# WangWen-Believer/DR-SLAM

Measured on AMD Instinct MI355X. Metric: RGB-D frames/sec (extract+match) at 640x480, higher is better.
Workload: dtype u8; 1 GPU; 640x480 synthetic RGB-D (TUM3 intrinsics), ORB extract 1000/1.2/8/20/7 + SearchByProjection(frame k, frame k-1, th=15) on consecutive frames; BASELINE config 2; batch_per_gpu=512, batches_in_flight_per_gpu=3, distinct_resident_input_batches_per_gpu=3, sequence_frames_per_rank=64

## Files before the change

### dr_slam_amd/csrc/match_kernels.hip

```cpp
#include "drfe_internal.h"
#include "match_internal.h"
#include "../../include/drfe_math.h"

#define WAVE 64


__global__ __launch_bounds__(256) void k_undistort(const drfe_keypoint* __restrict__ kps, const int* __restrict__ kpCount,
                                                   int maxKp, DrfeDistortion D, drfe_keypoint* __restrict__ kpsUn)
{
    const int slot = blockIdx.y;
    const int i = blockIdx.x * 256 + threadIdx.x;
    if (i >= kpCount[slot]) return;
    drfe_keypoint kp = kps[(size_t)slot * maxKp + i];
    float ux, uy;
    drfe_undistort_point(D, kp.x, kp.y, &ux, &uy);
    kp.x = ux; kp.y = uy;
    kpsUn[(size_t)slot * maxKp + i] = kp;
}

__global__ __launch_bounds__(256) void k_stereo(const drfe_keypoint* __restrict__ kps, const drfe_keypoint* __restrict__ kpsUn,
                                                const int* __restrict__ kpCount,
                                                int maxKp, const uint16_t* __restrict__ depth, size_t frameStride,
                                                size_t rowStride, int w, int h, drfe_camera cam,
                                                float* __restrict__ uRight, float* __restrict__ zDepth)
{
    const int slot = blockIdx.y;
    const int i = blockIdx.x * 256 + threadIdx.x;
    if (i >= kpCount[slot]) return;
    const drfe_keypoint kp = kps[(size_t)slot * maxKp + i];
    const int v = (int)kp.y, u = (int)kp.x;
    float d = 0.f;
    if (u >= 0 && u < w && v >= 0 && v < h)
        d = (float)depth[rowStride ? (size_t)slot * frameStride + (size_t)v * rowStride + u : (size_t)slot * frameStride + i] * cam.depth_factor;
    float ur = -1.f, z = -1.f;
    if (d > 0) { z = d; ur = kpsUn[(size_t)slot * maxKp + i].x - cam.bf / d; }
    uRight[(size_t)slot * maxKp + i] = ur;
    zDepth[(size_t)slot * maxKp + i] = z;
}

__device__ __forceinline__ int grid_cell(const drfe_keypoint& kp, const drfe_camera& cam, float invW, float invH)
{
    const int px = (int)roundf((kp.x - cam.min_x) * invW);
    const int py = (int)roundf((kp.y - cam.min_y) * invH);
    if (px < 0 || px >= DRFE_GRID_COLS || py < 0 || py >= DRFE_GRID_ROWS) return -1;
    return px * DRFE_GRID_ROWS + py;
}

__global__ __launch_bounds__(256) void k_grid(const drfe_keypoint* __restrict__ kps, const int* __restrict__ kpCount,
                                              int maxKp, drfe_camera cam, float invW, float invH,
                                              const float* __restrict__ uRight, const uint8_t* __restrict__ desc,
                                              int* __restrict__ gridOff, int* __restrict__ gridIdx,
                                              uint4* __restrict__ cellKp, uint4* __restrict__ cellDesc)
{
    __shared__ int cnt[DRFE_GRID_CELLS];
    __shared__ int off[DRFE_GRID_CELLS + 1];
    __shared__ int part[256];
    const int slot = blockIdx.x, tid = threadIdx.x;
    const int n = kpCount[slot];
    const drfe_keypoint* K = kps + (size_t)slot * maxKp;
    int* gIdx = gridIdx + (size_t)slot * maxKp;
    int* gOff = gridOff + (size_t)slot * (DRFE_GRID_CELLS + 1);
    for (int c = tid; c < DRFE_GRID_CELLS; c += 256) cnt[c] = 0;
    __syncthreads();
    for (int i = tid; i < n; i += 256) {
        const int c = grid_cell(K[i], cam, invW, invH);
        if (c >= 0) atomicAdd(&cnt[c], 1);
    }
    __syncthreads();
    const int per = DRFE_GRID_CELLS / 256;
    int s = 0;
    for (int k = 0; k < per; k++) s += cnt[tid * per + k];
    part[tid] = s;
    __syncthreads();
    for (int o = 1; o < 256; o <<= 1) {
        const int v = (tid >= o) ? part[tid - o] : 0;
        __syncthreads();
        part[tid] += v;
        __syncthreads();
    }
    int run = part[tid] - s;
    for (int k = 0; k < per; k++) { off[tid * per + k] = run; run += cnt[tid * per + k]; }
    if (tid == 255) off[DRFE_GRID_CELLS] = run;
    __syncthreads();
    for (int c = tid; c <= DRFE_GRID_CELLS; c += 256) gOff[c] = off[c];
    for (int c = tid; c < DRFE_GRID_CELLS; c += 256) cnt[c] = 0;
    __syncthreads();
    for (int i = tid; i < n; i += 256) {
        const int c = grid_cell(K[i], cam, invW, invH);
        if (c >= 0) gIdx[off[c] + atomicAdd(&cnt[c], 1)] = i;
    }
    __syncthreads();
    for (int c = tid; c < DRFE_GRID_CELLS; c += 256) {
        const int b = off[c], e = off[c + 1];
        for (int a = b + 1; a < e; a++) {
            const int v = gIdx[a];
            int j = a - 1;
            while (j >= b && gIdx[j] > v) { gIdx[j + 1] = gIdx[j]; j--; }
            gIdx[j + 1] = v;
        }
    }
    __syncthreads();
    const int nIn = off[DRFE_GRID_CELLS];
    uint4* cK = cellKp + (size_t)slot * maxKp;
    uint4* cD = cellDesc + (size_t)slot * maxKp * 2;
    const uint4* D4 = reinterpret_cast<const uint4*>(desc + (size_t)slot * maxKp * 32);
    const float* UR = uRight + (size_t)slot * maxKp;
    for (int p = tid; p < nIn; p += 256) {
        const int idx = gIdx[p];
        const drfe_keypoint kp = K[idx];
        cK[p] = make_uint4(__float_as_uint(kp.x), __float_as_uint(kp.y), __float_as_uint(UR[idx]),
                           (uint32_t)idx | ((uint32_t)kp.octave << 24));
        cD[2 * p] = D4[2 * idx];
        cD[2 * p + 1] = D4[2 * idx + 1];
    }
}


__device__ __forceinline__ void mat3_mul_add(const float* T , const float x[3], float out[3])
{
#pragma unroll
    for (int r = 0; r < 3; r++) {
        const float d = T[r * 4 + 0] * x[0] + T[r * 4 + 1] * x[1] + T[r * 4 + 2] * x[2];
        out[r] = d + T[r * 4 + 3];
    }
}

__global__ __launch_bounds__(256) void k_mappoints_last(const drfe_keypoint* __restrict__ kps,
                                                        const uint8_t* __restrict__ desc,
                                                        const int* __restrict__ kpCount, int maxKp,
                                                        const float* __restrict__ zDepth, drfe_camera cam,
                                                        const float* __restrict__ Twc ,
                                                        drfe_map_point* __restrict__ mps)
{
    const int slot = blockIdx.y;
    const int i = blockIdx.x * 256 + threadIdx.x;
    if (i >= kpCount[slot]) return;
    const size_t o = (size_t)slot * maxKp + i;
    drfe_map_point mp;
    const float z = zDepth[o];
    mp.valid = z > 0 ? 1 : 0;
    mp.obs_positive = 1;
    mp.pad[0] = mp.pad[1] = 0;
    mp.world[0] = mp.world[1] = mp.world[2] = 0.f;
    if (z > 0) {
        const float invfx = 1.0f / cam.fx, invfy = 1.0f / cam.fy;
        const drfe_keypoint kp = kps[o];
        float p[3];
        p[0] = (kp.x - cam.cx) * z * invfx;
        p[1] = (kp.y - cam.cy) * z * invfy;
        p[2] = z;
        mat3_mul_add(Twc + (size_t)slot * 16, p, mp.world);
    }
    const uint32_t* d = reinterpret_cast<const uint32_t*>(desc + o * 32);
    uint32_t* md = reinterpret_cast<uint32_t*>(mp.desc);
#pragma unroll
    for (int k = 0; k < 8; k++) md[k] = d[k];
    mps[o] = mp;
}

__global__ __launch_bounds__(256) void k_queries_last(const MatchPair* __restrict__ pairs,
                                                      const drfe_keypoint* __restrict__ kps,
                                                      const int* __restrict__ kpCount, int maxKp,
                                                      const drfe_map_point* __restrict__ mps, drfe_camera cam,
                                                      const float* __restrict__ scaleFactors, float th,
                                                      MatchQuery* __restrict__ queries)
{
    const MatchPair P = pairs[blockIdx.y];
    const int i = blockIdx.x * 256 + threadIdx.x;
    const int nLast = P.mpSlot >= 0 ? kpCount[P.lastSlot] : P.nQueries;
    if (i >= nLast) return;
    MatchQuery q;
    q.valid = 0;
    q.u = q.v = q.radius = q.ur = q.thrR = 0.f;
    q.minLevel = q.maxLevel = -1;
    q.obs = 0;
    const drfe_map_point mp = mps[(size_t)P.mpBase + i];
#pragma unroll
    for (int k = 0; k < 8; k++) q.desc[k] = reinterpret_cast<const uint32_t*>(mp.desc)[k];
    q.obs = mp.obs_positive;
    if (mp.valid) {
        float xc[3];
        mat3_mul_add(P.Tcw, mp.world, xc);
        const float invzc = (float)(1.0 / (double)xc[2]);
        if (!(invzc < 0)) {
            const float u = cam.fx * xc[0] * invzc + cam.cx;
            const float v = cam.fy * xc[1] * invzc + cam.cy;
            if (!(u < cam.min_x || u > cam.max_x) && !(v < cam.min_y || v > cam.max_y)) {
                const int oct = kps[(size_t)P.lastSlot * maxKp + i].octave;
                const float radius = th * scaleFactors[oct];
                q.u = u; q.v = v; q.radius = radius; q.thrR = radius;
                q.ur = u - cam.bf * invzc;
                if (P.forward) { q.minLevel = oct; q.maxLevel = -1; }
                else if (P.backward) { q.minLevel = 0; q.maxLevel = oct; }
                else { q.minLevel = oct - 1; q.maxLevel = oct + 1; }
                q.valid = 1;
            }
        }
    }
    queries[(size_t)P.queryBase + i] = q;
}


__device__ __forceinline__ bool window_cells(const MatchQuery& q, const drfe_camera& cam, float invW, float invH, int& minX,
                                             int& maxX, int& minY, int& maxY)
{
    const float x = q.u, y = q.v, r = q.radius;
    minX = max(0, (int)floorf((x - cam.min_x - r) * invW));
    maxX = min(DRFE_GRID_COLS - 1, (int)ceilf((x - cam.min_x + r) * invW));
    minY = max(0, (int)floorf((y - cam.min_y - r) * invH));
    maxY = min(DRFE_GRID_ROWS - 1, (int)ceilf((y - cam.min_y + r) * invH));
    return !(minX >= DRFE_GRID_COLS || maxX < 0 || minY >= DRFE_GRID_ROWS || maxY < 0);
}

__device__ __forceinline__ bool window_candidate(const MatchQuery& q, bool bCheckLevels, const uint4* __restrict__ cK,
                                                 const uint4* __restrict__ cD, int p, int sq, uint64_t q0, uint64_t q1,
                                                 uint64_t q2, uint64_t q3, uint32_t& key, uint32_t& id)
{
    const uint4 k4 = cK[p];
    const uint4 da = cD[2 * p], db = cD[2 * p + 1];
    const float kx = __uint_as_float(k4.x), ky = __uint_as_float(k4.y), ur = __uint_as_float(k4.z);
    const int oct = (int)(k4.w >> 24);
    bool ok = true;
    if (bCheckLevels) {
        if (oct < q.minLevel) ok = false;
        if (q.maxLevel >= 0 && oct > q.maxLevel) ok = false;
    }
    const float dx = kx - q.u, dy = ky - q.v;
    if (!(fabsf(dx) < q.radius && fabsf(dy) < q.radius)) ok = false;
    if (ur > 0) {
        const float er = fabsf(q.ur - ur);
        if (er > q.thrR) ok = false;
    }
    if (!ok) return false;
    const int dist = __popcll(q0 ^ ((uint64_t)da.x | ((uint64_t)da.y << 32))) + __popcll(q1 ^ ((uint64_t)da.z | ((uint64_t)da.w << 32))) +
                     __popcll(q2 ^ ((uint64_t)db.x | ((uint64_t)db.y << 32))) + __popcll(q3 ^ ((uint64_t)db.z | ((uint64_t)db.w << 32)));
    key = ((uint32_t)dist << 22) | (uint32_t)min(sq, (1 << 22) - 1);
    id = k4.w;
    return true;
}

__device__ void window_query_wave(const MatchQuery& q, size_t qo, int lane, int nMinCellX, int nMaxCellX, int nMinCellY, int nMaxCellY,
                                  const int* __restrict__ gOff, const uint4* __restrict__ cK, const uint4* __restrict__ cD,
                                  uint32_t* __restrict__ candIdx, uint32_t* __restrict__ candKey, int* __restrict__ candCnt,
                                  uint2* __restrict__ candBest, int* __restrict__ status)
{
    const bool bCheckLevels = (q.minLevel > 0) || (q.maxLevel >= 0);
    uint32_t* oIdx = candIdx + qo * DRFE_MATCH_MAX_CAND;
    uint32_t* oKey = candKey + qo * DRFE_MATCH_MAX_CAND;
    const uint64_t q0 = (uint64_t)q.desc[0] | ((uint64_t)q.desc[1] << 32), q1 = (uint64_t)q.desc[2] | ((uint64_t)q.desc[3] << 32),
                   q2 = (uint64_t)q.desc[4] | ((uint64_t)q.desc[5] << 32), q3 = (uint64_t)q.desc[6] | ((uint64_t)q.desc[7] << 32);
    const int ncol = nMaxCellX - nMinCellX + 1;
    int runB = 0, runN = 0;
    if (lane < ncol) {
        const int cb = (nMinCellX + lane) * DRFE_GRID_ROWS;
        runB = gOff[cb + nMinCellY];
        runN = gOff[cb + nMaxCellY + 1] - runB;
    }
    const int incl = drfe_wave_incl_scan(runN, lane);
    const int T = __builtin_amdgcn_readlane(incl, 63);
    int nOut = 0;
    bool overflow = false;
    uint32_t myKey = 0xFFFFFFFFu, myIdx = 0;
    for (int s0 = 0; s0 < T; s0 += WAVE) {
        const int sq = s0 + lane;
        bool pass = false;
        uint32_t key = 0xFFFFFFFFu, id = 0;
        int base = __builtin_amdgcn_readfirstlane(runB);
        for (int j = 0; j + 1 < ncol; j++) {
            const int inclJ = __builtin_amdgcn_readlane(incl, j), nextB = __builtin_amdgcn_readlane(runB, j + 1);
            if (inclJ <= sq) base = nextB - inclJ;
        }
        if (sq < T) pass = window_candidate(q, bCheckLevels, cK, cD, base + sq, sq, q0, q1, q2, q3, key, id);
        const unsigned long long m = __ballot(pass);
        const int pos = nOut + __popcll(m & ((1ull << lane) - 1ull));
        if (pass) {
            if (pos < DRFE_MATCH_MAX_CAND) {
                oIdx[pos] = id;
                oKey[pos] = key;
                if (key < myKey) { myKey = key; myIdx = id; }
            } else overflow = true;
        }
        nOut += __popcll(m);
    }
    if (__any(overflow) && lane == 0) atomicOr(status, 4);
    const uint32_t mn = drfe_wave_min_u32(myKey);
    const unsigned long long who = __ballot(myKey == mn);
    const uint32_t bIdx = (uint32_t)__builtin_amdgcn_readlane((int)myIdx, __ffsll((long long)who) - 1);
    if (lane == 0) {
        candCnt[qo] = min(nOut, DRFE_MATCH_MAX_CAND);
        candBest[qo] = make_uint2(mn, bIdx);
    }
}

#define WQ_TAB 64
#ifndef WQ_THREADS
#define WQ_THREADS 64
#endif
#define WQ_PER_BLOCK (WQ_THREADS / WAVE * 4)
__global__ __launch_bounds__(WQ_THREADS) void k_window_candidates(const MatchPair* __restrict__ pairs,
                                                           const MatchQuery* __restrict__ queries,
                                                           const int* __restrict__ kpCount, int maxKp,
                                                           const int* __restrict__ gridOff,
                                                           const uint4* __restrict__ cellKp,
                                                           const uint4* __restrict__ cellDesc, drfe_camera cam,
                                                           float invW, float invH,
                                                           uint32_t* __restrict__ candIdx,
                                                           uint32_t* __restrict__ candKey,
                                                           int* __restrict__ candCnt, uint2* __restrict__ candBest,
                                                           int* __restrict__ status, uint32_t gxMagic)
{
    __shared__ int sTab[WQ_THREADS / WAVE][4][WQ_TAB];
    int bx, by;
    drfe_xcd_swizzle_2d(gxMagic, bx, by);
    const MatchPair P = pairs[by];
    const int wv = __builtin_amdgcn_readfirstlane((int)(threadIdx.x >> 6)), lane = threadIdx.x & 63;
    const int g = lane >> 4, l = lane & 15;
    const int qbase = (bx * (WQ_THREADS / WAVE) + wv) * 4;
    const int nQ = P.mpSlot >= 0 ? kpCount[P.lastSlot] : P.nQueries;
    if (qbase >= nQ) return;
    const int cur = P.curSlot;
    const int* gOff = gridOff + (size_t)cur * (DRFE_GRID_CELLS + 1);
    const uint4* cK = cellKp + (size_t)cur * maxKp;
    const uint4* cD = cellDesc + (size_t)cur * maxKp * 2;
    const bool have = qbase + g < nQ;
    const size_t qo = (size_t)P.queryBase + (have ? qbase + g : qbase);
    const MatchQuery q = queries[qo];
    int nMinCellX = 0, nMaxCellX = 0, nMinCellY = 0, nMaxCellY = 0;
    const bool inRange = have && q.valid && window_cells(q, cam, invW, invH, nMinCellX, nMaxCellX, nMinCellY, nMaxCellY);
    const int ncol = nMaxCellX - nMinCellX + 1;
    int runB = 0, runN = 0;
    const bool narrow = inRange && ncol <= 16;
    if (narrow && l < ncol) {
        const int cb = (nMinCellX + l) * DRFE_GRID_ROWS;
        runB = gOff[cb + nMinCellY];
        runN = gOff[cb + nMaxCellY + 1] - runB;
    }
    int incl = runN;
    incl += __builtin_amdgcn_update_dpp(0, incl, 0x111, 0xf, 0xf, true);
    incl += __builtin_amdgcn_update_dpp(0, incl, 0x112, 0xf, 0xf, true);
    incl += __builtin_amdgcn_update_dpp(0, incl, 0x114, 0xf, 0xf, true);
    incl += __builtin_amdgcn_update_dpp(0, incl, 0x118, 0xf, 0xf, true);
    const int T = __shfl(incl, 15, 16);
    const bool small = narrow && T <= WQ_TAB;
    {
        const int excl = incl - runN;
        const int n = small ? runN : 0;
        for (int k = 0; __any(k < n); k++)
            if (k < n) sTab[wv][g][excl + k] = runB + k;
    }
    const bool bCheckLevels = (q.minLevel > 0) || (q.maxLevel >= 0);
    const uint64_t q0 = (uint64_t)q.desc[0] | ((uint64_t)q.desc[1] << 32), q1 = (uint64_t)q.desc[2] | ((uint64_t)q.desc[3] << 32),
                   q2 = (uint64_t)q.desc[4] | ((uint64_t)q.desc[5] << 32), q3 = (uint64_t)q.desc[6] | ((uint64_t)q.desc[7] << 32);
    uint32_t* oIdx = candIdx + qo * DRFE_MATCH_MAX_CAND;
    uint32_t* oKey = candKey + qo * DRFE_MATCH_MAX_CAND;
    const int Tg = small ? T : 0;
    int nOut = 0;
    uint32_t myKey = 0xFFFFFFFFu, myIdx = 0;
    for (int s0 = 0; __any(s0 < Tg); s0 += 16) {
        const int sq = s0 + l;
        bool pass = false;
        uint32_t key = 0xFFFFFFFFu, id = 0;
        if (sq < Tg) pass = window_candidate(q, bCheckLevels, cK, cD, sTab[wv][g][sq], sq, q0, q1, q2, q3, key, id);
        const uint32_t m16 = (uint32_t)(__ballot(pass) >> (g * 16)) & 0xFFFFu;
        const int pos = nOut + __popc(m16 & ((1u << l) - 1u));
        if (pass) {
            oIdx[pos] = id;
            oKey[pos] = key;
            if (key < myKey) { myKey = key; myIdx = id; }
        }
        nOut += __popc(m16);
    }
    uint32_t mn = myKey;
    mn = min(mn, (uint32_t)__builtin_amdgcn_update_dpp((int)mn, (int)mn, 0xB1, 0xf, 0xf, false));
    mn = min(mn, (uint32_t)__builtin_amdgcn_update_dpp((int)mn, (int)mn, 0x4E, 0xf, 0xf, false));
    mn = min(mn, (uint32_t)__builtin_amdgcn_update_dpp((int)mn, (int)mn, 0x141, 0xf, 0xf, false));
    mn = min(mn, (uint32_t)__builtin_amdgcn_update_dpp((int)mn, (int)mn, 0x140, 0xf, 0xf, false));
    const uint32_t who16 = (uint32_t)(__ballot(myKey == mn) >> (g * 16)) & 0xFFFFu;
    const uint32_t bIdx = (uint32_t)__shfl((int)myIdx, __ffs((int)who16) - 1, 16);
    if (have && l == 0 && (small || !inRange)) {
        candCnt[qo] = nOut;
        candBest[qo] = small ? make_uint2(mn, bIdx) : make_uint2(0xFFFFFFFFu, 0u);
    }
    unsigned long long wide = __ballot(inRange && !small && l == 0);
    while (wide) {
        const int gg = (__ffsll((long long)wide) - 1) >> 4;
        wide &= wide - 1;
        const size_t qw = (size_t)P.queryBase + qbase + gg;
        const MatchQuery qq = queries[qw];
        int x0, x1, y0, y1;
        window_cells(qq, cam, invW, invH, x0, x1, y0, y1);
        window_query_wave(qq, qw, lane, x0, x1, y0, y1, gOff, cK, cD, candIdx, candKey, candCnt, candBest, status);
    }
}


__device__ __forceinline__ uint32_t wave_min_u32(uint32_t v) { return drfe_wave_min_u32(v); }

#define RS_THREADS 512
#define RS_MAX_T 8
static_assert(RS_THREADS * RS_MAX_T == DRFE_MATCH_LAST_MAX_QUERIES, "the C-ABI checks this limit before launching");
__global__ __launch_bounds__(RS_THREADS) void k_resolve_last(const MatchPair* __restrict__ pairs,
                                                             const MatchQuery* __restrict__ queries,
                                                             const drfe_keypoint* __restrict__ kps,
                                                             const int* __restrict__ kpCount, int maxKp,
                                                             const uint32_t* __restrict__ candIdx,
                                                             const uint32_t* __restrict__ candKey,
                                                             const int* __restrict__ candCnt,
                                                             const uint2* __restrict__ candBest, int checkOri,
                                                             int* __restrict__ match ,
                                                             const uint8_t* __restrict__ initObs,
                                                             int* __restrict__ matchCount,
                                                             uint16_t* __restrict__ histScratch )
{
    extern __shared__ int rs_smem[];
    int* owner = rs_smem;
    unsigned char* claim = reinterpret_cast<unsigned char*>(rs_smem + maxKp);
    __shared__ int hist[30];
    __shared__ int sNm, sEnt, sInd[3], sChanged[3];
    const MatchPair P = pairs[blockIdx.x];
    const int tid = threadIdx.x;
    const int nQ = P.mpSlot >= 0 ? kpCount[P.lastSlot] : P.nQueries;
    const int nCur = kpCount[P.curSlot];
    int* M = match + (size_t)P.curSlot * maxKp;
    const drfe_keypoint* Kc = kps + (size_t)P.curSlot * maxKp;
    const drfe_keypoint* Kl = kps + (size_t)P.lastSlot * maxKp;
    uint16_t* hs = histScratch + (size_t)blockIdx.x * 2 * maxKp;
    for (int i = tid; i < nCur; i += RS_THREADS) {
        unsigned char c = 0;
        if (M[i] >= 0) c = 1 | ((initObs ? initObs[i] : 1) ? 2 : 0);
        claim[i] = c;
    }
    if (tid < 30) hist[tid] = 0;
    if (tid == 0) { sNm = 0; sEnt = 0; sChanged[0] = 0; }
    const float factor = 1.0f / 30;
    int cnt[RS_MAX_T], obs[RS_MAX_T];
    uint32_t bKey[RS_MAX_T], bIdx[RS_MAX_T], pKey[RS_MAX_T], pIdx[RS_MAX_T];
#pragma unroll
    for (int t = 0; t < RS_MAX_T; t++) {
        const int i = tid + t * RS_THREADS;
        cnt[t] = 0; obs[t] = 0; bKey[t] = 0xFFFFFFFFu; bIdx[t] = 0; pKey[t] = 0xFFFFFFFFu; pIdx[t] = 0;
        if (i < nQ) {
            const size_t qo = (size_t)P.queryBase + i;
            cnt[t] = candCnt[qo];
            if (cnt[t] > 0) { const uint2 b = candBest[qo]; bKey[t] = b.x; bIdx[t] = b.y; obs[t] = queries[qo].obs; }
        }
    }
    for (int sweep = 0;; sweep++) {
        for (int k = tid; k < nCur; k += RS_THREADS) owner[k] = 0x7FFFFFFF;
        if (tid == 0) sChanged[(sweep + 1) % 3] = 0;
        __syncthreads();
#pragma unroll
        for (int t = 0; t < RS_MAX_T; t++)
            if (obs[t] && pKey[t] != 0xFFFFFFFFu && (int)(pKey[t] >> 22) <= 100)
                atomicMin(&owner[pIdx[t] & 0xFFFFFF], tid + t * RS_THREADS);
        __syncthreads();
        bool changed = false;
#pragma unroll
        for (int t = 0; t < RS_MAX_T; t++) {
            if (cnt[t] == 0) continue;
            const int i = tid + t * RS_THREADS;
            uint32_t key = 0xFFFFFFFFu, idx = 0;
            const int kb = (int)(bIdx[t] & 0xFFFFFF);
            if ((claim[kb] & 3) != 3 && owner[kb] >= i) { key = bKey[t]; idx = bIdx[t]; }
            else {
                const size_t qo = ((size_t)P.queryBase + i) * DRFE_MATCH_MAX_CAND;
                for (int j0 = 0; j0 < cnt[t]; j0 += 8) {
                    const uint4 ka = *reinterpret_cast<const uint4*>(candKey + qo + j0);
                    const uint4 kb2 = *reinterpret_cast<const uint4*>(candKey + qo + j0 + 4);
                    const uint4 ia = *reinterpret_cast<const uint4*>(candIdx + qo + j0);
                    const uint4 ib = *reinterpret_cast<const uint4*>(candIdx + qo + j0 + 4);
                    const uint32_t kv[8] = {ka.x, ka.y, ka.z, ka.w, kb2.x, kb2.y, kb2.z, kb2.w};
                    const uint32_t iv[8] = {ia.x, ia.y, ia.z, ia.w, ib.x, ib.y, ib.z, ib.w};
#pragma unroll
                    for (int u = 0; u < 8; u++) {
                        if (j0 + u >= cnt[t] || kv[u] >= key) continue;
                        const int kk = (int)(iv[u] & 0xFFFFFF);
                        if ((claim[kk] & 3) != 3 && owner[kk] >= i) { key = kv[u]; idx = iv[u]; }
                    }
                }
            }
            if (key != pKey[t] || idx != pIdx[t]) { changed = true; pKey[t] = key; pIdx[t] = idx; }
        }
        if (changed) sChanged[sweep % 3] = 1;
        __syncthreads();
        if (!__builtin_amdgcn_readfirstlane(sChanged[sweep % 3])) break;
    }
    for (int k = tid; k < nCur; k += RS_THREADS) owner[k] = -1;
    __syncthreads();
#pragma unroll
    for (int t = 0; t < RS_MAX_T; t++) {
        if (pKey[t] == 0xFFFFFFFFu || (int)(pKey[t] >> 22) > 100) continue;
        const int i = tid + t * RS_THREADS;
        const int i2 = (int)(pIdx[t] & 0xFFFFFF);
        atomicMax(&owner[i2], i);
        atomicAdd(&sNm, 1);
        if (checkOri) {
            float rot = Kl[i].angle - Kc[i2].angle;
            if (rot < 0.0f) rot += 360.0f;
            int bin = (int)roundf(rot * factor);
            if (bin == 30) bin = 0;
            const int e = atomicAdd(&sEnt, 1);
            hs[2 * e] = (uint16_t)bin;
            hs[2 * e + 1] = (uint16_t)i2;
            atomicAdd(&hist[bin], 1);
        }
    }
    __syncthreads();
    for (int k = tid; k < nCur; k += RS_THREADS)
        if (owner[k] >= 0) M[k] = owner[k];
    __syncthreads();
    if (checkOri) {
        if (tid == 0) {
            int max1 = 0, max2 = 0, max3 = 0, ind1 = -1, ind2 = -1, ind3 = -1;
            for (int i = 0; i < 30; i++) {
                const int s = hist[i];
                if (s > max1) { max3 = max2; max2 = max1; max1 = s; ind3 = ind2; ind2 = ind1; ind1 = i; }
                else if (s > max2) { max3 = max2; max2 = s; ind3 = ind2; ind2 = i; }
                else if (s > max3) { max3 = s; ind3 = i; }
            }
            if (max2 < 0.1f * (float)max1) { ind2 = -1; ind3 = -1; }
            else if (max3 < 0.1f * (float)max1) { ind3 = -1; }
            sInd[0] = ind1; sInd[1] = ind2; sInd[2] = ind3;
        }
        __syncthreads();
        const int nEnt = sEnt;
        for (int e = tid; e < nEnt; e += RS_THREADS) {
            const int bin = hs[2 * e];
            if (bin != sInd[0] && bin != sInd[1] && bin != sInd[2]) { M[hs[2 * e + 1]] = -1; atomicSub(&sNm, 1); }
        }
        __syncthreads();
    }
    if (tid == 0) matchCount[P.curSlot] = sNm;
}

__global__ __launch_bounds__(WAVE) void k_resolve_map(const MatchPair* __restrict__ pairs,
                                                      const MatchQuery* __restrict__ queries,
                                                      const int* __restrict__ kpCount, int maxKp,
                                                      const uint32_t* __restrict__ candIdx,
                                                      const uint32_t* __restrict__ candKey,
                                                      const int* __restrict__ candCnt, float nnratio,
                                                      int* __restrict__ match, const uint8_t* __restrict__ initObs,
                                                      int* __restrict__ matchCount)
{
    extern __shared__ unsigned char claim[];
    const MatchPair P = pairs[blockIdx.x];
    const int lane = threadIdx.x;
    const int nQ = P.nQueries;
    const int nCur = kpCount[P.curSlot];
    int* M = match + (size_t)P.curSlot * maxKp;
    for (int i = lane; i < nCur; i += WAVE) {
        unsigned char c = 0;
        if (M[i] >= 0) c = 1 | ((initObs ? initObs[i] : 1) ? 2 : 0);
        claim[i] = c;
    }
    __syncthreads();
    int nmatches = 0;
    for (int i = 0; i < nQ; i++) {
        const size_t qo = (size_t)P.queryBase + i;
        const int cnt = candCnt[qo];
        if (cnt == 0) continue;
        uint32_t k1 = 0xFFFFFFFFu, i1 = 0, k2 = 0xFFFFFFFFu, i2 = 0;
        for (int c0 = 0; c0 < cnt; c0 += WAVE) {
            uint32_t key = 0xFFFFFFFFu, idx = 0;
            if (c0 + lane < cnt) {
                idx = candIdx[qo * DRFE_MATCH_MAX_CAND + c0 + lane];
                key = candKey[qo * DRFE_MATCH_MAX_CAND + c0 + lane];
                if ((claim[idx & 0xFFFFFF] & 3) == 3) key = 0xFFFFFFFFu;
            }
            for (int pass = 0; pass < 2; pass++) {
                const uint32_t mn = wave_min_u32(key);
                if (mn == 0xFFFFFFFFu) break;
                const unsigned long long who = __ballot(key == mn);
                const int src = __ffsll((long long)who) - 1;
                const uint32_t ix = (uint32_t)__shfl((int)idx, src);
                if (mn < k1) { k2 = k1; i2 = i1; k1 = mn; i1 = ix; }
                else if (mn < k2) { k2 = mn; i2 = ix; }
                if (lane == src) key = 0xFFFFFFFFu;
            }
        }
        if (k1 == 0xFFFFFFFFu) continue;
        const int bestDist = (int)(k1 >> 22);
        const int bestDist2 = (k2 == 0xFFFFFFFFu) ? 256 : (int)(k2 >> 22);
        const int bestLevel = (int)(i1 >> 24);
        const int bestLevel2 = (k2 == 0xFFFFFFFFu) ? -1 : (int)(i2 >> 24);
        if (bestDist <= 100) {
            if (bestLevel == bestLevel2 && (float)bestDist > nnratio * (float)bestDist2) continue;
            const int bi = (int)(i1 & 0xFFFFFF);
            if (lane == 0) { M[bi] = i; claim[bi] = 1 | (queries[qo].obs ? 2 : 0); }
            nmatches++;
            __syncthreads();
        }
    }
    if (lane == 0) matchCount[P.curSlot] = nmatches;
}


__global__ __launch_bounds__(64) void k_bf_knn(const uint8_t* __restrict__ Q, int nq, const uint8_t* __restrict__ T,
                                               int nt, int k, int* __restrict__ outIdx, int* __restrict__ outDist)
{
    __shared__ uint64_t tile[64 * 4];
    const int lane = threadIdx.x;
    const int qi = blockIdx.x * 64 + lane;
    uint64_t q[4] = {0, 0, 0, 0};
    if (qi < nq) {
        const uint64_t* p = reinterpret_cast<const uint64_t*>(Q + (size_t)qi * 32);
        q[0] = p[0]; q[1] = p[1]; q[2] = p[2]; q[3] = p[3];
    }
    int d1 = 1 << 30, i1 = -1, d2 = 1 << 30, i2 = -1;
    for (int t0 = 0; t0 < nt; t0 += 64) {
        __syncthreads();
        if (t0 + lane < nt) {
            const uint64_t* p = reinterpret_cast<const uint64_t*>(T + (size_t)(t0 + lane) * 32);
            tile[lane * 4 + 0] = p[0]; tile[lane * 4 + 1] = p[1]; tile[lane * 4 + 2] = p[2]; tile[lane * 4 + 3] = p[3];
        }
        __syncthreads();
        const int m = min(64, nt - t0);
        for (int j = 0; j < m; j++) {
            const int d = __popcll(q[0] ^ tile[j * 4]) + __popcll(q[1] ^ tile[j * 4 + 1]) +
                          __popcll(q[2] ^ tile[j * 4 + 2]) + __popcll(q[3] ^ tile[j * 4 + 3]);
            if (d < d1) { d2 = d1; i2 = i1; d1 = d; i1 = t0 + j; }
            else if (d < d2) { d2 = d; i2 = t0 + j; }
        }
    }
    if (qi < nq) {
        outIdx[(size_t)qi * k] = i1;
        outDist[(size_t)qi * k] = i1 >= 0 ? d1 : -1;
        if (k > 1) {
            outIdx[(size_t)qi * k + 1] = i2;
            outDist[(size_t)qi * k + 1] = i2 >= 0 ? d2 : -1;
        }
    }
}



__global__ __launch_bounds__(256) void k_kp_pixels(const drfe_keypoint* __restrict__ kps, const int* __restrict__ kpCount, int maxKp,
                                                   int w, int h, uint32_t* __restrict__ uv)
{
    const int slot = blockIdx.y;
    const int i = blockIdx.x * 256 + threadIdx.x;
    if (i >= maxKp) return;
    uint32_t o = 0xFFFFFFFFu;
    if (i < kpCount[slot]) {
        const drfe_keypoint kp = kps[(size_t)slot * maxKp + i];
        const int v = (int)kp.y, u = (int)kp.x;
        if (u >= 0 && u < w && v >= 0 && v < h) o = (uint32_t)u | ((uint32_t)v << 16);
    }
    uv[(size_t)slot * maxKp + i] = o;
}

hipError_t drfe_launch_kp_pixels(drfe_ctx* c, int nframes, uint32_t* d_uv, hipStream_t s)
{
    hipLaunchKernelGGL(k_kp_pixels, dim3((c->maxKp + 255) / 256, nframes), dim3(256), 0, s, c->d_kps, c->d_kpCount, c->maxKp,
                       c->geom.imgW, c->geom.imgH, d_uv);
    return hipGetLastError();
}

hipError_t drfe_launch_glue(drfe_ctx* c, const uint16_t* d_depth, size_t frameStride, size_t rowStride,
                            const drfe_camera& cam, int nframes, hipStream_t s)
{
    const float invW = (float)DRFE_GRID_COLS / (float)(cam.max_x - cam.min_x);
    const float invH = (float)DRFE_GRID_ROWS / (float)(cam.max_y - cam.min_y);
    prof_begin(c, DRFE_STAGE_GLUE, s);
    if (c->dist.enabled)
        hipLaunchKernelGGL(k_undistort, dim3((c->maxKp + 255) / 256, nframes), dim3(256), 0, s, c->d_kps, c->d_kpCount,
// ... 578 lines not shown
```

Before: 303,500 frames/s.

## Rebuild grid binning in LDS with rank sort; replace window table with bpermute search

k_grid now computes each keypoint's cell once into LDS, scans the cell counts with a wave-level scan into 16-bit offsets, and orders each cell's members by rank counting in LDS instead of an insertion sort on global memory. The packed cell arrays are then built from the LDS sorted list, and global gIdx is written alongside them. The old path is kept as a fallback when maxKp exceeds the LDS capacity. In k_window_candidates the per-wave shared sTab table is replaced by a 4-step binary search over the lanes' inclusive prefix sums via ds_bpermute, which removes the shared memory and its fill loop but adds permute work on every candidate iteration.

```diff
diff --git a/dr_slam_amd/csrc/match_kernels.hip b/dr_slam_amd/csrc/match_kernels.hip
--- a/dr_slam_amd/csrc/match_kernels.hip
+++ b/dr_slam_amd/csrc/match_kernels.hip
@@ -46,20 +46,26 @@
     return px * DRFE_GRID_ROWS + py;
 }
 
-__global__ __launch_bounds__(256) void k_grid(const drfe_keypoint* __restrict__ kps, const int* __restrict__ kpCount,
-                                              int maxKp, drfe_camera cam, float invW, float invH,
-                                              const float* __restrict__ uRight, const uint8_t* __restrict__ desc,
-                                              int* __restrict__ gridOff, int* __restrict__ gridIdx,
-                                              uint4* __restrict__ cellKp, uint4* __restrict__ cellDesc)
-{
-    __shared__ int cnt[DRFE_GRID_CELLS];
-    __shared__ int off[DRFE_GRID_CELLS + 1];
-    __shared__ int part[256];
-    const int slot = blockIdx.x, tid = threadIdx.x;
-    const int n = kpCount[slot];
-    const drfe_keypoint* K = kps + (size_t)slot * maxKp;
-    int* gIdx = gridIdx + (size_t)slot * maxKp;
-    int* gOff = gridOff + (size_t)slot * (DRFE_GRID_CELLS + 1);
+template <typename I>
+__device__ __forceinline__ void grid_pack_cells(const I* idx, int nIn, const drfe_keypoint* __restrict__ K,
+                                                const float* __restrict__ UR, const uint4* __restrict__ D4,
+                                                int* __restrict__ gIdx, uint4* __restrict__ cK, uint4* __restrict__ cD, int tid)
+{
+    for (int p = tid; p < nIn; p += 256) {
+        const int i = (int)idx[p];
+        const drfe_keypoint kp = K[i];
+        if (gIdx) gIdx[p] = i;
+        cK[p] = make_uint4(__float_as_uint(kp.x), __float_as_uint(kp.y), __float_as_uint(UR[i]),
+                           (uint32_t)i | ((uint32_t)kp.octave << 24));
+        cD[2 * p] = D4[2 * i];
+        cD[2 * p + 1] = D4[2 * i + 1];
+    }
+}
+
+__device__ void grid_lists_global(const drfe_keypoint* __restrict__ K, int n, const drfe_camera& cam, float invW, float invH,
+                                  int* __restrict__ gOff, int* __restrict__ gIdx, int* cnt, int* off, int* part)
+{
+    const int tid = threadIdx.x;
     for (int c = tid; c < DRFE_GRID_CELLS; c += 256) cnt[c] = 0;
     __syncthreads();
     for (int i = tid; i < n; i += 256) {
@@ -100,19 +106,93 @@
         }
     }
     __syncthreads();
-    const int nIn = off[DRFE_GRID_CELLS];
+}
+
+#define GRID_LDS_KP 4096
+#define GRID_OFF16_BYTES ((DRFE_GRID_CELLS + 1) * 2 + 14)
+#define GRID_LDS_BYTES (DRFE_GRID_CELLS * 4 + GRID_OFF16_BYTES + 2 * GRID_LDS_KP * 2)
+static_assert(GRID_OFF16_BYTES % 16 == 0 && DRFE_GRID_CELLS % (256 * 4) == 0, "k_grid's LDS sections are 16-byte aligned, 12 cells per thread");
+static_assert(GRID_LDS_BYTES >= DRFE_GRID_CELLS * 4 + (DRFE_GRID_CELLS + 4) * 4 + 256 * 4, "grid_lists_global's arrays fit the same block");
+static_assert(GRID_LDS_BYTES + 16 <= 40 * 1024, "the workgroup has to fit beside the other batches' kernels");
+__global__ __launch_bounds__(256) void k_grid(const drfe_keypoint* __restrict__ kps, const int* __restrict__ kpCount,
+                                              int maxKp, drfe_camera cam, float invW, float invH,
+                                              const float* __restrict__ uRight, const uint8_t* __restrict__ desc,
+                                              int* __restrict__ gridOff, int* __restrict__ gridIdx,
+                                              uint4* __restrict__ cellKp, uint4* __restrict__ cellDesc)
+{
+    __shared__ __align__(16) unsigned char lds[GRID_LDS_BYTES];
+    __shared__ int wtot[4];
+    const int slot = blockIdx.x, tid = threadIdx.x;
+    const int n = min(kpCount[slot], maxKp);
+    const drfe_keypoint* K = kps + (size_t)slot * maxKp;
+    int* gIdx = gridIdx + (size_t)slot * maxKp;
+    int* gOff = gridOff + (size_t)slot * (DRFE_GRID_CELLS + 1);
     uint4* cK = cellKp + (size_t)slot * maxKp;
     uint4* cD = cellDesc + (size_t)slot * maxKp * 2;
     const uint4* D4 = reinterpret_cast<const uint4*>(desc + (size_t)slot * maxKp * 32);
     const float* UR = uRight + (size_t)slot * maxKp;
-    for (int p = tid; p < nIn; p += 256) {
-        const int idx = gIdx[p];
-        const drfe_keypoint kp = K[idx];
-        cK[p] = make_uint4(__float_as_uint(kp.x), __float_as_uint(kp.y), __float_as_uint(UR[idx]),
-                           (uint32_t)idx | ((uint32_t)kp.octave << 24));
-        cD[2 * p] = D4[2 * idx];
-        cD[2 * p + 1] = D4[2 * idx + 1];
-    }
+    int* cur = reinterpret_cast<int*>(lds);
+    if (maxKp > GRID_LDS_KP) {
+        int* off = cur + DRFE_GRID_CELLS;
+        grid_lists_global(K, n, cam, invW, invH, gOff, gIdx, cur, off, off + DRFE_GRID_CELLS + 4);
+        grid_pack_cells(gIdx, off[DRFE_GRID_CELLS], K, UR, D4, (int*)nullptr, cK, cD, tid);
+        return;
+    }
+    uint16_t* off = reinterpret_cast<uint16_t*>(lds + DRFE_GRID_CELLS * 4);
+    uint16_t* cell = reinterpret_cast<uint16_t*>(lds + DRFE_GRID_CELLS * 4 + GRID_OFF16_BYTES);
+    uint16_t* lst = cell + GRID_LDS_KP;
+    uint16_t* sorted = reinterpret_cast<uint16_t*>(lds);
+    const int per = DRFE_GRID_CELLS / 256;
+    uint4* mine = reinterpret_cast<uint4*>(cur + tid * per);
+    mine[0] = mine[1] = mine[2] = make_uint4(0, 0, 0, 0);
+    for (int i = tid; i < n; i += 256) cell[i] = (uint16_t)grid_cell(K[i], cam, invW, invH);
+    __syncthreads();
+    for (int i = tid; i < n; i += 256) {
+        const int c = cell[i];
+        if (c != 0xFFFF) atomicAdd(&cur[c], 1);
+    }
+    __syncthreads();
+    const uint4 c0 = mine[0], c1 = mine[1], c2 = mine[2];
+    const int v[12] = {(int)c0.x, (int)c0.y, (int)c0.z, (int)c0.w, (int)c1.x, (int)c1.y, (int)c1.z, (int)c1.w,
+                       (int)c2.x, (int)c2.y, (int)c2.z, (int)c2.w};
+    int s = 0;
+#pragma unroll
+    for (int k = 0; k < per; k++) s += v[k];
+    const int incl = drfe_wave_incl_scan(s, tid & 63);
+    if ((tid & 63) == 63) wtot[tid >> 6] = incl;
+    __syncthreads();
+    int run = incl - s;
+#pragma unroll
+    for (int w = 0; w < 3; w++) run += (tid >> 6) > w ? wtot[w] : 0;
+    {
+        int e[12];
+#pragma unroll
+        for (int k = 0; k < per; k++) { e[k] = run; run += v[k]; }
+        mine[0] = make_uint4(e[0], e[1], e[2], e[3]);
+        mine[1] = make_uint4(e[4], e[5], e[6], e[7]);
+        mine[2] = make_uint4(e[8], e[9], e[10], e[11]);
+        uint32_t* o2 = reinterpret_cast<uint32_t*>(off) + tid * (per / 2);
+#pragma unroll
+        for (int k = 0; k < per / 2; k++) o2[k] = (uint32_t)e[2 * k] | ((uint32_t)e[2 * k + 1] << 16);
+        if (tid == 255) off[DRFE_GRID_CELLS] = (uint16_t)run;
+    }
+    __syncthreads();
+    for (int c = tid; c <= DRFE_GRID_CELLS; c += 256) gOff[c] = off[c];
+    for (int i = tid; i < n; i += 256) {
+        const int c = cell[i];
+        if (c != 0xFFFF) lst[atomicAdd(&cur[c], 1)] = (uint16_t)i;
+    }
+    __syncthreads();
+    for (int i = tid; i < n; i += 256) {
+        const int c = cell[i];
+        if (c == 0xFFFF) continue;
+        const int b = off[c], e = off[c + 1];
+        int rank = 0;
+        for (int p = b; p < e; p++) rank += lst[p] < i;
+        sorted[b + rank] = (uint16_t)i;
+    }
+    __syncthreads();
+    grid_pack_cells(sorted, (int)off[DRFE_GRID_CELLS], K, UR, D4, gIdx, cK, cD, tid);
 }
 
 
@@ -309,7 +389,6 @@
                                                            int* __restrict__ candCnt, uint2* __restrict__ candBest,
                                                            int* __restrict__ status, uint32_t gxMagic)
 {
-    __shared__ int sTab[WQ_THREADS / WAVE][4][WQ_TAB];
     int bx, by;
     drfe_xcd_swizzle_2d(gxMagic, bx, by);
     const MatchPair P = pairs[by];
@@ -342,12 +421,8 @@
     incl += __builtin_amdgcn_update_dpp(0, incl, 0x118, 0xf, 0xf, true);
     const int T = __shfl(incl, 15, 16);
     const bool small = narrow && T <= WQ_TAB;
-    {
-        const int excl = incl - runN;
-        const int n = small ? runN : 0;
-        for (int k = 0; __any(k < n); k++)
-            if (k < n) sTab[wv][g][excl + k] = runB + k;
-    }
+    const int adj = runB - (incl - runN);
+    const int row4 = (lane & 48) << 2;
     const bool bCheckLevels = (q.minLevel > 0) || (q.maxLevel >= 0);
     const uint64_t q0 = (uint64_t)q.desc[0] | ((uint64_t)q.desc[1] << 32), q1 = (uint64_t)q.desc[2] | ((uint64_t)q.desc[3] << 32),
                    q2 = (uint64_t)q.desc[4] | ((uint64_t)q.desc[5] << 32), q3 = (uint64_t)q.desc[6] | ((uint64_t)q.desc[7] << 32);
@@ -360,7 +435,13 @@
         const int sq = s0 + l;
         bool pass = false;
         uint32_t key = 0xFFFFFFFFu, id = 0;
-        if (sq < Tg) pass = window_candidate(q, bCheckLevels, cK, cD, sTab[wv][g][sq], sq, q0, q1, q2, q3, key, id);
+        int j = 0;
+        j += __builtin_amdgcn_ds_bpermute(row4 + ((j + 7) << 2), incl) <= sq ? 8 : 0;
+        j += __builtin_amdgcn_ds_bpermute(row4 + ((j + 3) << 2), incl) <= sq ? 4 : 0;
+        j += __builtin_amdgcn_ds_bpermute(row4 + ((j + 1) << 2), incl) <= sq ? 2 : 0;
+        j += __builtin_amdgcn_ds_bpermute(row4 + (j << 2), incl) <= sq ? 1 : 0;
+        const int rec = sq + __builtin_amdgcn_ds_bpermute(row4 + (j << 2), adj);
+        if (sq < Tg) pass = window_candidate(q, bCheckLevels, cK, cD, rec, sq, q0, q1, q2, q3, key, id);
         const uint32_t m16 = (uint32_t)(__ballot(pass) >> (g * 16)) & 0xFFFFu;
         const int pos = nOut + __popc(m16 & ((1u << l) - 1u));
         if (pass) {
```

Result: no change. 303,700 frames/s, median of 4 (+0.1%).
